# real-stanford/flingbot

Measured on AMD Instinct MI355X. Metric: sim steps/sec (64x64-particle cloth), higher is better.
Workload: dtype f32

## Files before the change

### flingbot_amd/csrc/fs_fused_grid_kernel.h

```cpp
#pragma once
#include "fs_fused_kernel.h"

#define FG_PLANE (FS_FUSED_MAX_PARTICLES * 4)
#define FG_PAD 1024
#define FG_OFF_XX FG_PAD
#define FG_OFF_X0 (FG_OFF_XX + 4 * FG_PLANE)
#define FG_OFF_CACC (FG_OFF_X0 + 3 * FG_PLANE)
#define FG_OFF_CUR (FG_OFF_CACC + FS_FUSED_CSET_CAP * 16)
#define FG_OFF_ITEMS (FG_OFF_CUR + FS_FUSED_CUR_BYTES)
#define FG_OFF_SCAN (FG_OFF_ITEMS + FS_FUSED_MAX_PARTICLES * 2)
#define FG_OFF_CSET (FG_OFF_SCAN + 64)
#define FG_OFF_CHIST (FG_OFF_CSET + FS_FUSED_CSET_CAP * 2)
#define FG_OFF_ROWL (FG_OFF_CHIST + 512)
#define FG_OFF_KZ (FG_OFF_ROWL + 1024)
#define FG_OFF_KS (FG_OFF_KZ + 1024)
#define FG_OFF_COLL (FG_OFF_KS + 1024)
#define FG_OFF_RCNT (FG_OFF_COLL + 512)
#define FG_LDS_BYTES (FG_OFF_RCNT + 512)
static_assert(FG_OFF_ROWL % 8 == 0 && (FG_OFF_KZ - FG_OFF_ROWL) % 8 == 0, "row tables are read as ds_read_b64 pairs");
static_assert((FG_OFF_COLL - FG_OFF_KS) % 256 == 0, "column tables share one address, rows as ds_read2st64_b32 offsets");
static_assert(FG_LDS_BYTES <= 160 * 1024, "grid-64 kernel: the LDS of one CU");
static_assert(FG_OFF_CACC % 16 == 0 && FG_OFF_CUR == FG_OFF_CACC + FS_FUSED_CSET_CAP * 16, "set and queue accumulators: one array");
#ifndef FG_SINGLES
#define FG_SINGLES 1
#endif
#define FG_SINGLES_LANES (FS_FUSED_THREADS - 64)
#define FG_SINGLES_ROOM ((FS_FUSED_CUR_BYTES + FS_FUSED_MAX_PARTICLES * 2) / 16)
#define FG_SINGLES_CAP (FG_SINGLES_ROOM < 2 * FG_SINGLES_LANES ? FG_SINGLES_ROOM : 2 * FG_SINGLES_LANES)
#define FG_SLOT_NONE 0xffffu
#define FG_SLOT_INLINE 0xfffeu
static_assert(FS_FUSED_CSET_CAP + FG_SINGLES_CAP <= FG_SLOT_INLINE, "slot values below the reserved ones");

#define FG_ROW(w, k) (2 * (w) + 32 * ((k) >> 1) + ((k) & 1))

template <int DZ>
__device__ __forceinline__ void fg_load_slot(unsigned a, fs_f2 &x0, fs_f2 &x1, fs_f2 &x2) {
    asm volatile("ds_read2st64_b32 %0, %1 offset0:%2 offset1:%3" : "=v"(x0) : "v"(a), "n"(DZ + 2), "n"(DZ + 3) : "memory");
    asm volatile("ds_read2st64_b32 %0, %1 offset0:%2 offset1:%3" : "=v"(x1) : "v"(a), "n"(DZ + 2 + 64), "n"(DZ + 3 + 64) : "memory");
    asm volatile("ds_read2st64_b32 %0, %1 offset0:%2 offset1:%3" : "=v"(x2) : "v"(a), "n"(DZ + 2 + 128), "n"(DZ + 3 + 128) : "memory");
}
template <int OFF>
__device__ __forceinline__ fs_f2 fg_load_rows(unsigned a) {
    static_assert(OFF >= 0 && OFF < 65536 && OFF % 8 == 0, "ds_read_b64 offset");
    fs_f2 r;
    asm volatile("ds_read_b64 %0, %1 offset:%2" : "=v"(r) : "v"(a), "n"(OFF) : "memory");
    return r;
}
template <int R0, int R1>
__device__ __forceinline__ fs_f2 fg_load_cols(unsigned a) {
    static_assert(R0 >= 0 && R0 < 256 && R1 >= 0 && R1 < 256, "ds_read2st64_b32 offsets");
    fs_f2 r;
    asm volatile("ds_read2st64_b32 %0, %1 offset0:%2 offset1:%3" : "=v"(r) : "v"(a), "n"(R0), "n"(R1) : "memory");
    return r;
}
#define FG_WAIT(N, A0, A1, A2) asm volatile("s_waitcnt lgkmcnt(" #N ")" : "+v"(A0), "+v"(A1), "+v"(A2))

#define FG_MIN_L2 1.17549435e-38f
__device__ __forceinline__ float fg_scale(float xi0, float xi1, float xi2, float xj0, float xj1, float xj2, float L, float k,
                                          float &l2) {
    const float ex = xi0 - xj0, ey = xi1 - xj1, ez = xi2 - xj2;
    l2 = fs_dot3(ex, ey, ez, ex, ey, ez);
    const float inv = __builtin_amdgcn_rsqf(l2);
    const float len = l2 * inv;
    const float C = len - L;
    return k * (C * inv);
}
__device__ __forceinline__ void fg_accum(float &d0, float &d1, float &d2, float xi0, float xi1, float xi2, float xj0, float xj1,
                                         float xj2, float sc) {
    const float ex = xi0 - xj0, ey = xi1 - xj1, ez = xi2 - xj2;
    d0 = FS_FMA(-ex, sc, d0);
    d1 = FS_FMA(-ey, sc, d1);
    d2 = FS_FMA(-ez, sc, d2);
}
__device__ __forceinline__ float fg_from_left(float v) {
    return __int_as_float(__builtin_amdgcn_update_dpp(0, __float_as_int(v), 0x138, 0xf, 0xf, true));
}
__device__ __forceinline__ float fg_from_right(float v) {
    return __int_as_float(__builtin_amdgcn_update_dpp(0, __float_as_int(v), 0x130, 0xf, 0xf, true));
}

__device__ __forceinline__ void fg_apply(const FsAcc &a, float relax, const float *rcnt, float &x0, float &x1, float &x2) {
    if (a.cnt > 0) {
        const float sc = a.cnt < 128 ? rcnt[a.cnt] : relax / (float)a.cnt;
        x0 = FS_FMA(a.d0, sc, x0); x1 = FS_FMA(a.d1, sc, x1); x2 = FS_FMA(a.d2, sc, x2);
    }
}

__global__ __launch_bounds__(FS_FUSED_THREADS) void fs_k_fused_grid64(const FsEnvDev *__restrict__ envs,
                                                                      const FsShapesDev *__restrict__ shapes, const int *ids,
                                                                      int n_steps) {
    static_assert(FS_FUSED_THREADS == 1024 && FS_FUSED_PPT == 4, "grid-64 kernel: 16 waves x 4 rows");
    extern __shared__ __attribute__((aligned(16))) char smem[];
    float *Xx = (float *)(smem + FG_OFF_XX);
    float *Xy = Xx + FS_FUSED_MAX_PARTICLES, *Xz = Xy + FS_FUSED_MAX_PARTICLES, *Xw = Xz + FS_FUSED_MAX_PARTICLES;
    float *X0x = (float *)(smem + FG_OFF_X0);
    float *X0y = X0x + FS_FUSED_MAX_PARTICLES;
    float *X0z = X0y + FS_FUSED_MAX_PARTICLES;
    unsigned short *cursor = (unsigned short *)(smem + FG_OFF_CUR);
    unsigned short *items = (unsigned short *)(smem + FG_OFF_ITEMS);
    int *wave_tot = (int *)(smem + FG_OFF_SCAN);
    float *rowL = (float *)(smem + FG_OFF_ROWL);

#ifdef FS_BLOCK_CLOCKS
    const unsigned long long tc_start = __builtin_amdgcn_s_memtime(), tr_start = __builtin_amdgcn_s_memrealtime();
#endif
#ifdef FS_TIMING
    unsigned long long ts_acc[16] = {0, 0, 0, 0, 0, 0, 0, 0, 0, 0, 0, 0, 0, 0, 0, 0};
    unsigned long long ts_last = __builtin_amdgcn_s_memtime();
#endif
    const int e = ids[blockIdx.x];
    if (e < 0) return;
    const FsEnvDev &E = envs[e];
    const FsShapesDev &sh = shapes[e];
    const FsFusedConsts c = fs_fused_consts(E, sh);
    const int n = c.n;
    const unsigned un = (unsigned)n;
    const int t = threadIdx.x, lane = t & 63, w = t >> 6;
    const int dimz = n >> 6;

    FsVec4 *const g_pos = E.pos, *const g_vel = E.vel;
    const FsVec4 *const g_rest = E.rest;
    const fs_gci g_phase = (fs_gci)E.phase;
    const fs_gi g_nlist = (fs_gi)E.nlist, g_ncount = (fs_gi)E.ncount;
    const fs_gci g_ell_j = (fs_gci)E.ell_j;
    const fs_gcf g_ell_len = (fs_gcf)E.ell_len, g_ell_k = (fs_gcf)E.ell_k;
    const fs_gcf g_L = (fs_gcf)E.g64_L;
    const int max_deg = E.max_deg;
    const fs_gcu g_near = (fs_gcu)E.restnear_w;

    int find_mode = 0;
    {
        const int ph0 = g_phase[0];
        int differs = 0;
        for (int i = t; i < n; i += FS_FUSED_THREADS) differs |= (g_phase[i] != ph0);
        if (t == 0) wave_tot[0] = 0;
        __syncthreads();
        if (differs) atomicOr(&wave_tot[0], 1);
        __syncthreads();
        const int mixed = wave_tot[0];
        __syncthreads();
        if (!mixed) {
            if (!(ph0 & FS_PHASE_SELF_COLLIDE)) find_mode = 3;
            else if (!(ph0 & FS_PHASE_SELF_COLLIDE_FILTER)) find_mode = 2;
            else if (E.restnear_ok == 2 && FS_STENCIL_FILTER) find_mode = 4;
            else if (E.restnear_ok) find_mode = 1;
        }
    }
    for (int q = t; q < FG_OFF_X0 / 4; q += FS_FUSED_THREADS) ((float *)smem)[q] = 0.0f;
    __syncthreads();
    for (int i = t; i < n; i += FS_FUSED_THREADS) {
        const FsVec4 p = fs_ld4(g_pos, i);
        Xx[i] = p.x; Xy[i] = p.y; Xz[i] = p.z; Xw[i] = p.w;
        X0x[i] = p.x; X0y[i] = p.y; X0z[i] = p.z;
    }
    if (t < 256) {
        const int r = t & 63, s = 8 + (t >> 6);
        rowL[t] = r < dimz ? g_L[(unsigned)s * un + (unsigned)(r * 64 + 2)] : 0.0f;
    }
    constexpr int XS_DX[4] = {-1, -2, +1, +2};
    constexpr int SH_DX[4] = {+1, -1, -1, +1}, SH_DZ[4] = {-1, -1, +1, +1};
    constexpr int ZS_DZ[4] = {-1, -2, +1, +2};
    float *colL = (float *)(smem + FG_OFF_COLL);
    if (t < 128) {
        const int col = t & 63, q = t >> 6;
        const int dxq = q == 0 ? -1 : -2;
        colL[t] = (unsigned)(col + dxq) < 64u ? g_L[(unsigned)q * un + (unsigned)(2 * 64 + col)] : 0.0f;
    }
    float *rcnt = (float *)(smem + FG_OFF_RCNT);
    if (t < 128) rcnt[t] = t > 0 ? c.relax / (float)t : 0.0f;
    if (t < 256) {
        const int c64 = t & 63, q = t >> 6;
        const int sdx = (q == 0 || q == 3) ? +1 : -1, sslot = q < 2 ? 2 + q : 4 + q;
        const int zdz = q < 2 ? -1 - q : q - 1;
        ((float *)(smem + FG_OFF_KS))[t] = (unsigned)(c64 + sdx) < 64u ? E.g64_kh[sslot] : 0.0f;
        ((float *)(smem + FG_OFF_KZ))[t] = (c64 < dimz && (unsigned)(c64 + zdz) < (unsigned)dimz) ? E.g64_kh[8 + q] : 0.0f;
    }
    const float kh0 = E.g64_kh[0], kh1 = E.g64_kh[1];
    unsigned nvalid = 0u;
#pragma unroll
    for (int k = 0; k < FS_FUSED_PPT; ++k) {
        const int row = FG_ROW(w, k);
        int cnt = 0;
#pragma unroll
        for (int q = 0; q < 4; ++q) {
            cnt += ((unsigned)(lane + XS_DX[q]) < 64u) ? 1 : 0;
            cnt += ((unsigned)(lane + SH_DX[q]) < 64u && (unsigned)(row + SH_DZ[q]) < (unsigned)dimz) ? 1 : 0;
            cnt += ((unsigned)(row + ZS_DZ[q]) < (unsigned)dimz) ? 1 : 0;
        }
        nvalid |= (unsigned)cnt << (8 * k);
    }
    __syncthreads();
    unsigned fastmask = 0u;
    {
        constexpr int cdx[FS_G64_SLOTS] = FS_G64_DX_LIST, cdz[FS_G64_SLOTS] = FS_G64_DZ_LIST;
#pragma unroll
        for (int k = 0; k < FS_FUSED_PPT; ++k) {
            const int row = FG_ROW(w, k), i = row * 64 + lane;
            bool differs = false;
            if (i < n) {
                const float wi = Xw[i];
                differs = !(wi > 0.0f);
#pragma unroll
                for (int q = 0; q < FS_G64_SLOTS; ++q) {
                    const bool in = (unsigned)(lane + cdx[q]) < 64u && (unsigned)(row + cdz[q]) < (unsigned)dimz;
                    if (in) differs |= Xw[i + cdz[q] * 64 + cdx[q]] != wi;
                }
            }
            if (i < n && __builtin_amdgcn_ballot_w64(differs) == 0ull) fastmask |= 1u << k;
        }
        fastmask = (unsigned)__builtin_amdgcn_readfirstlane((int)fastmask);
    }

    FS_TS(0)
#pragma unroll 1
    for (int frame = 0; frame < n_steps; ++frame) {
#pragma unroll 1
        for (int sub = 0; sub < c.substeps; ++sub) {
            for (int q = t; q < FS_FUSED_BUCKETS / 2; q += FS_FUSED_THREADS) ((unsigned *)cursor)[q] = 0u;
            FsVec4 xp[FS_FUSED_PPT];
#pragma unroll
            for (int k = 0; k < FS_FUSED_PPT; ++k) {
                const int i = t + k * FS_FUSED_THREADS;
                xp[k] = FsVec4{0.0f, 0.0f, 0.0f, 0.0f};
                if (i < n) {
                    const FsVec4 p0 = FsVec4{X0x[i], X0y[i], X0z[i], Xw[i]};
                    xp[k] = fs_fused_predict(c, p0, fs_ld4(g_vel, i));
                    fs_st4(E.x0, i, p0);
                }
            }
            __syncthreads();
            fs_fused_build_grid(c, xp, cursor, items, wave_tot, X0x, X0y, X0z);
            FS_TS(1)
            const FsFindConsts fc = {n, c.ncap, c.rad2, c.inv_rad, find_mode, E.gp_dimx, E.gp_magic};
#pragma unroll 1
            for (int qs = t; qs < n; qs += FS_FUSED_THREADS) {
                const int i = items[qs];
                const FsVec4 xi = FsVec4{X0x[qs], X0y[qs], X0z[qs], 0.0f};
                const int shape_bits = (int)(fs_shape_candidates(E.p, sh, sub, xi.x, xi.y, xi.z) << FS_SHAPE_MASK_SHIFT);
                if (find_mode == 4) {
                    FsNearWords none;
#pragma unroll
                    for (int q = 0; q < 8; ++q) none.w[q] = 0xffffffffu;
                    g_ncount[i] = fs_fused_find_neighbors<true>(fc, i, xi, (fs_lcus)cursor, (fs_lcus)items, g_phase, g_rest, g_nlist,
                                                                none, (fs_lus)(smem + FG_OFF_XX) + t, (fs_lcf)X0x) | shape_bits;
                    continue;
                }
                FsNearWords near;
#pragma unroll
                for (int q = 0; q < 8; ++q) near.w[q] = find_mode == 1 ? g_near[(unsigned)q * un + (unsigned)i] : 0xffffffffu;
                g_ncount[i] = (find_mode == 3 ? 0
                                              : fs_fused_find_neighbors<false>(fc, i, xi, (fs_lcus)cursor, (fs_lcus)items, g_phase,
                                                                               g_rest, g_nlist, near,
                                                                               (fs_lus)(smem + FG_OFF_XX) + t, (fs_lcf)X0x)) |
                              shape_bits;
            }
            FS_TS(2)
            __syncthreads();
            FS_TS(3)
#pragma unroll
            for (int k = 0; k < FS_FUSED_PPT; ++k) {
                const int i = t + k * FS_FUSED_THREADS;
                if (i < n) {
                    Xx[i] = xp[k].x; Xy[i] = xp[k].y; Xz[i] = xp[k].z; Xw[i] = xp[k].w;
                    const FsVec4 p0 = fs_ld4(E.x0, i);
                    X0x[i] = p0.x; X0y[i] = p0.y; X0z[i] = p0.z;
                } else {
                    Xx[i] = 0.0f; Xy[i] = 0.0f; Xz[i] = 0.0f; Xw[i] = 0.0f;
                }
            }

            unsigned short *cset = (unsigned short *)(smem + FG_OFF_CSET);
            FsVec4 *cacc = (FsVec4 *)(smem + FG_OFF_CACC);
            int *chist = (int *)(smem + FG_OFF_CHIST);
            if (t < 128) chist[t] = 0;
            int *nsingles = (int *)(smem + FG_OFF_SCAN);
            if (t == 0) *nsingles = 0;
            __syncthreads();
            int ccls[FS_FUSED_PPT];
#pragma unroll
            for (int k = 0; k < FS_FUSED_PPT; ++k) {
                const int i = FG_ROW(w, k) * 64 + lane;
                int cc = 0;
                if (i < n && Xw[i] > 0.0f) cc = g_ncount[i] & FS_NCOUNT_MASK;
                ccls[k] = cc > 96 ? 96 : cc;
                if (ccls[k] > 0) atomicAdd(&chist[ccls[k]], 1);
            }
            __syncthreads();
            fs_fused_count_offsets(chist, t);
            __syncthreads();
            FsVec4 *squeue = cacc + FS_FUSED_CSET_CAP;
            unsigned long long slotpack = ~0ull;
#pragma unroll
            for (int k = 0; k < FS_FUSED_PPT; ++k) {
                if (ccls[k] > 0) {
                    const int i = FG_ROW(w, k) * 64 + lane;
                    unsigned slot = FG_SLOT_INLINE;
                    const int pos = atomicAdd(&chist[ccls[k]], 1);
                    if (pos < FS_FUSED_CSET_CAP) {
                        cset[pos] = (unsigned short)i;
                        slot = (unsigned)pos;
                    }
#if FG_SINGLES
                    else if (ccls[k] <= 16) {
                        const int sp = atomicAdd(nsingles, 1);
                        if (sp < FG_SINGLES_CAP) {
                            slot = (unsigned)(FS_FUSED_CSET_CAP + sp);
                            squeue[sp].w = __int_as_float(i | (g_nlist[i] << 12) | ((ccls[k] - 1) << 28));
                        }
                    }
#endif
                    slotpack = (slotpack & ~(0xffffull << (16 * k))) | ((unsigned long long)slot << (16 * k));
                }
            }
            __syncthreads();
            const int csize = chist[0] < FS_FUSED_CSET_CAP ? chist[0] : FS_FUSED_CSET_CAP;
            const int n_singles = *nsingles < FG_SINGLES_CAP ? *nsingles : FG_SINGLES_CAP;
            const int i2 = t < csize ? (int)cset[t] : -1;
            int cnt2 = 0, cj2[FS_FUSED_PREFETCH_CAND];
#pragma unroll
            for (int q = 0; q < FS_FUSED_PREFETCH_CAND; ++q) cj2[q] = 0;
            if (i2 >= 0) {
                cnt2 = g_ncount[i2] & FS_NCOUNT_MASK;
#pragma unroll
                for (int q = 0; q < FS_FUSED_PREFETCH_CAND; ++q) cj2[q] = g_nlist[(unsigned)q * un + (unsigned)i2];
            }
            static_assert(FG_SINGLES_CAP <= 2 * FG_SINGLES_LANES, "two queue entries per lane");
            unsigned qw0 = 0u, qw1 = 0u;
#if FG_SINGLES
            if (t >= 64 && t - 64 < n_singles) qw0 = (unsigned)__float_as_int(squeue[t - 64].w);
            if (t >= 64 && t - 64 + FG_SINGLES_LANES < n_singles) qw1 = (unsigned)__float_as_int(squeue[t - 64 + FG_SINGLES_LANES].w);
            __syncthreads();
#endif

            FS_TS(4)
#pragma unroll 1
            for (int it = 0; it < c.iters; ++it) {
                unsigned cpack = 0u;
                float rx[FS_FUSED_PPT], ry[FS_FUSED_PPT], rz[FS_FUSED_PPT];
#pragma unroll
                for (int q = 0; q < FS_FUSED_PPT; ++q) { rx[q] = 0.0f; ry[q] = 0.0f; rz[q] = 0.0f; }
#ifdef FG_UNROLL_PAIRS
#pragma unroll
#else
#pragma unroll 1
#endif
                for (int pr = 0; pr < 2; ++pr) {
                    const int rowP = FG_ROW(w, 2 * pr);
                    const int iP_raw = rowP * 64 + lane, iQ_raw = iP_raw + 64;
                    const bool haveP = rowP < dimz, haveQ = rowP + 1 < dimz;
                    const int iP = haveP ? iP_raw : 0, iQ = haveQ ? iQ_raw : 0;
                    const bool fast = haveQ && ((fastmask >> (2 * pr)) & 3u) == 3u;
                    const fs_f2 xi0 = fs_f2{Xx[iP], Xx[iQ]}, xi1 = fs_f2{Xy[iP], Xy[iQ]}, xi2 = fs_f2{Xz[iP], Xz[iQ]};
                    const fs_f2 wi = fs_f2{Xw[iP], Xw[iQ]};
                    FsAcc aP, aQ;
                    bool exact = !fast;
                    if (fast) {
                        unsigned aLane = (unsigned)(lane * 4);
                        asm volatile("" : "+v"(aLane));
                        const unsigned am2 = (unsigned)(FG_OFF_XX + ((rowP - 2) * 64 - 2) * 4) + aLane;
                        const unsigned am1 = am2 + 4u, a00 = am2 + 8u, ap1 = am2 + 12u, ap2 = am2 + 16u;
                        constexpr int SH_SLOT[4] = {2, 3, 6, 7};
                        float sLP[2], sLQ[4];
#pragma unroll
                        for (int q = 0; q < 2; ++q) sLP[q] = g_L[(unsigned)SH_SLOT[q] * un + (unsigned)iP];
#pragma unroll
                        for (int q = 0; q < 4; ++q) sLQ[q] = g_L[(unsigned)SH_SLOT[q] * un + (unsigned)iQ];
                        const unsigned aRow = (unsigned)(FG_OFF_ROWL + rowP * 4), aCol = (unsigned)FG_OFF_KS + aLane;
                        constexpr int CL_ROW = (FG_OFF_COLL - FG_OFF_KS) / 256;
                        fs_f2 cL = fg_load_cols<CL_ROW, CL_ROW + 1>(aCol);
                        const unsigned aKP = rowP >= 1 ? aCol : aLane;
                        const unsigned aKQ = rowP + 2 < dimz ? aCol : aLane;
                        fs_f2 kP23 = fg_load_cols<0, 1>(aKP);
                        fs_f2 kQ23 = fg_load_cols<0, 1>(aCol);
#define FG_KX(q) ((unsigned)(lane + XS_DX[q]) < 64u ? (q == 0 ? kh0 : kh1) : 0.0f)
                        float dP0 = 0.0f, dP1 = 0.0f, dP2 = 0.0f, dQ0 = 0.0f, dQ1 = 0.0f, dQ2 = 0.0f, mP = 1.0f, mQ = 1.0f;
                        fs_f2 u0, u1, u2, v0, v1, v2;
                        float l2a, l2b, l2c, l2d;
                        fg_load_slot<0>(am1, u0, u1, u2);
                        fg_load_slot<0>(am2, v0, v1, v2);
                        asm volatile("s_waitcnt lgkmcnt(3)"
                                     : "+v"(cL), "+v"(kP23), "+v"(kQ23), "+v"(u0), "+v"(u1), "+v"(u2));
                        const float scP0 = fg_scale(xi0.x, xi1.x, xi2.x, u0.x, u1.x, u2.x, cL.x, FG_KX(0), l2a);
                        const float scQ0 = fg_scale(xi0.y, xi1.y, xi2.y, u0.y, u1.y, u2.y, cL.x, FG_KX(0), l2b);
                        fg_accum(dP0, dP1, dP2, xi0.x, xi1.x, xi2.x, u0.x, u1.x, u2.x, scP0);
                        fg_accum(dQ0, dQ1, dQ2, xi0.y, xi1.y, xi2.y, u0.y, u1.y, u2.y, scQ0);
                        __builtin_amdgcn_sched_barrier(0);
                        fg_load_slot<-1>(ap1, u0, u1, u2);
                        FG_WAIT(3, v0, v1, v2);
                        const float scP1 = fg_scale(xi0.x, xi1.x, xi2.x, v0.x, v1.x, v2.x, cL.y, FG_KX(1), l2c);
                        const float scQ1 = fg_scale(xi0.y, xi1.y, xi2.y, v0.y, v1.y, v2.y, cL.y, FG_KX(1), l2d);
                        fg_accum(dP0, dP1, dP2, xi0.x, xi1.x, xi2.x, v0.x, v1.x, v2.x, scP1);
                        fg_accum(dQ0, dQ1, dQ2, xi0.y, xi1.y, xi2.y, v0.y, v1.y, v2.y, scQ1);
                        mP = fminf(fminf(mP, l2a), l2c);
                        mQ = fminf(fminf(mQ, l2b), l2d);
                        __builtin_amdgcn_sched_barrier(0);
                        fg_load_slot<-1>(am1, v0, v1, v2);
                        FG_WAIT(3, u0, u1, u2);
                        const float scQ2 = fg_scale(xi0.y, xi1.y, xi2.y, u0.y, u1.y, u2.y, sLQ[0], kQ23.x, l2b);
                        {
                            const float sc = fg_scale(xi0.x, xi1.x, xi2.x, u0.x, u1.x, u2.x, sLP[0], kP23.x, l2a);
                            fg_accum(dP0, dP1, dP2, xi0.x, xi1.x, xi2.x, u0.x, u1.x, u2.x, sc);
                        }
                        fg_accum(dQ0, dQ1, dQ2, xi0.y, xi1.y, xi2.y, u0.y, u1.y, u2.y, scQ2);
                        __builtin_amdgcn_sched_barrier(0);
                        fg_load_slot<0>(ap1, u0, u1, u2);
                        FG_WAIT(3, v0, v1, v2);
                        const float scQ3 = fg_scale(xi0.y, xi1.y, xi2.y, v0.y, v1.y, v2.y, sLQ[1], kQ23.y, l2d);
                        {
                            const float sc = fg_scale(xi0.x, xi1.x, xi2.x, v0.x, v1.x, v2.x, sLP[1], kP23.y, l2c);
                            fg_accum(dP0, dP1, dP2, xi0.x, xi1.x, xi2.x, v0.x, v1.x, v2.x, sc);
                        }
                        fg_accum(dQ0, dQ1, dQ2, xi0.y, xi1.y, xi2.y, v0.y, v1.y, v2.y, scQ3);
                        mP = fminf(fminf(mP, l2a), l2c);
                        mQ = fminf(fminf(mQ, l2b), l2d);
                        __builtin_amdgcn_sched_barrier(0);
                        fg_load_slot<0>(ap2, v0, v1, v2);
                        FG_WAIT(3, u0, u1, u2);
                        fg_accum(dP0, dP1, dP2, xi0.x, xi1.x, xi2.x, u0.x, u1.x, u2.x, fg_from_right(scP0));
                        fg_accum(dQ0, dQ1, dQ2, xi0.y, xi1.y, xi2.y, u0.y, u1.y, u2.y, fg_from_right(scQ0));
                        __builtin_amdgcn_sched_barrier(0);
                        fs_f2 kQ67 = fg_load_cols<2, 3>(aKQ);
                        fg_load_slot<+1>(am1, u0, u1, u2);
                        FG_WAIT(3, v0, v1, v2);
                        fg_accum(dP0, dP1, dP2, xi0.x, xi1.x, xi2.x, v0.x, v1.x, v2.x, fg_from_right(fg_from_right(scP1)));
                        fg_accum(dQ0, dQ1, dQ2, xi0.y, xi1.y, xi2.y, v0.y, v1.y, v2.y, fg_from_right(fg_from_right(scQ1)));
                        __builtin_amdgcn_sched_barrier(0);
                        fg_load_slot<+1>(ap1, v0, v1, v2);
                        asm volatile("s_waitcnt lgkmcnt(3)" : "+v"(kQ67), "+v"(u0), "+v"(u1), "+v"(u2));
                        fg_accum(dP0, dP1, dP2, xi0.x, xi1.x, xi2.x, u0.x, u1.x, u2.x, fg_from_left(scQ2));
                        {
                            const float sc = fg_scale(xi0.y, xi1.y, xi2.y, u0.y, u1.y, u2.y, sLQ[2], kQ67.x, l2a);
                            fg_accum(dQ0, dQ1, dQ2, xi0.y, xi1.y, xi2.y, u0.y, u1.y, u2.y, sc);
                        }
                        __builtin_amdgcn_sched_barrier(0);
                        constexpr int KZ = FG_OFF_KZ - FG_OFF_ROWL;
                        fs_f2 zL[4], zK[4];
                        zL[0] = fg_load_rows<0>(aRow); zK[0] = fg_load_rows<KZ>(aRow);
                        zL[1] = fg_load_rows<256>(aRow); zK[1] = fg_load_rows<KZ + 256>(aRow);
                        fg_load_slot<-1>(a00, u0, u1, u2);
                        asm volatile("s_waitcnt lgkmcnt(3)"
                                     : "+v"(zL[0]), "+v"(zK[0]), "+v"(zL[1]), "+v"(zK[1]), "+v"(v0), "+v"(v1), "+v"(v2));
                        fg_accum(dP0, dP1, dP2, xi0.x, xi1.x, xi2.x, v0.x, v1.x, v2.x, fg_from_right(scQ3));
                        {
                            const float sc = fg_scale(xi0.y, xi1.y, xi2.y, v0.y, v1.y, v2.y, sLQ[3], kQ67.y, l2b);
                            fg_accum(dQ0, dQ1, dQ2, xi0.y, xi1.y, xi2.y, v0.y, v1.y, v2.y, sc);
                        }
                        mQ = fminf(fminf(mQ, l2a), l2b);
                        __builtin_amdgcn_sched_barrier(0);
                        fg_load_slot<-2>(a00, v0, v1, v2);
                        FG_WAIT(3, u0, u1, u2);
                        const float scQ8 = fg_scale(xi0.y, xi1.y, xi2.y, u0.y, u1.y, u2.y, zL[0].y, zK[0].y, l2b);
                        {
                            const float sc = fg_scale(xi0.x, xi1.x, xi2.x, u0.x, u1.x, u2.x, zL[0].x, zK[0].x, l2a);
                            fg_accum(dP0, dP1, dP2, xi0.x, xi1.x, xi2.x, u0.x, u1.x, u2.x, sc);
                        }
                        fg_accum(dQ0, dQ1, dQ2, xi0.y, xi1.y, xi2.y, u0.y, u1.y, u2.y, scQ8);
                        __builtin_amdgcn_sched_barrier(0);
                        zL[2] = fg_load_rows<512>(aRow); zK[2] = fg_load_rows<KZ + 512>(aRow);
                        zL[3] = fg_load_rows<768>(aRow); zK[3] = fg_load_rows<KZ + 768>(aRow);
                        fg_load_slot<+1>(a00, u0, u1, u2);
                        asm volatile("s_waitcnt lgkmcnt(3)"
                                     : "+v"(zL[2]), "+v"(zK[2]), "+v"(zL[3]), "+v"(zK[3]), "+v"(v0), "+v"(v1), "+v"(v2));
                        {
                            const float sc = fg_scale(xi0.x, xi1.x, xi2.x, v0.x, v1.x, v2.x, zL[1].x, zK[1].x, l2c);
                            const float sd = fg_scale(xi0.y, xi1.y, xi2.y, v0.y, v1.y, v2.y, zL[1].y, zK[1].y, l2d);
                            fg_accum(dP0, dP1, dP2, xi0.x, xi1.x, xi2.x, v0.x, v1.x, v2.x, sc);
                            fg_accum(dQ0, dQ1, dQ2, xi0.y, xi1.y, xi2.y, v0.y, v1.y, v2.y, sd);
                        }
                        mP = fminf(fminf(mP, l2a), l2c);
                        mQ = fminf(fminf(mQ, l2b), l2d);
                        __builtin_amdgcn_sched_barrier(0);
                        fg_load_slot<+2>(a00, v0, v1, v2);
                        FG_WAIT(3, u0, u1, u2);
                        fg_accum(dP0, dP1, dP2, xi0.x, xi1.x, xi2.x, u0.x, u1.x, u2.x, scQ8);
                        {
                            const float sd = fg_scale(xi0.y, xi1.y, xi2.y, u0.y, u1.y, u2.y, zL[2].y, zK[2].y, l2c);
                            fg_accum(dQ0, dQ1, dQ2, xi0.y, xi1.y, xi2.y, u0.y, u1.y, u2.y, sd);
                        }
                        __builtin_amdgcn_sched_barrier(0);
                        FG_WAIT(0, v0, v1, v2);
                        {
                            const float sc = fg_scale(xi0.x, xi1.x, xi2.x, v0.x, v1.x, v2.x, zL[3].x, zK[3].x, l2a);
                            const float sd = fg_scale(xi0.y, xi1.y, xi2.y, v0.y, v1.y, v2.y, zL[3].y, zK[3].y, l2b);
                            fg_accum(dP0, dP1, dP2, xi0.x, xi1.x, xi2.x, v0.x, v1.x, v2.x, sc);
                            fg_accum(dQ0, dQ1, dQ2, xi0.y, xi1.y, xi2.y, v0.y, v1.y, v2.y, sd);
                        }
                        mP = fminf(mP, l2a);
                        mQ = fminf(fminf(mQ, l2c), l2b);
                        __builtin_amdgcn_sched_barrier(0);
#undef FG_KX
                        exact = __builtin_amdgcn_ballot_w64(mP < FG_MIN_L2 || mQ < FG_MIN_L2) != 0ull;
                        aP = FsAcc{dP0, dP1, dP2, (int)((nvalid >> (16 * pr)) & 0xffu)};
                        aQ = FsAcc{dQ0, dQ1, dQ2, (int)((nvalid >> (16 * pr + 8)) & 0xffu)};
                    }
                    if (exact) {
                        aP = FsAcc{0.0f, 0.0f, 0.0f, 0};
                        aQ = FsAcc{0.0f, 0.0f, 0.0f, 0};
                        if (haveP && wi.x > 0.0f)
                            for (int s = 0; s < max_deg; ++s) {
                                const int j = g_ell_j[(unsigned)s * un + (unsigned)iP];
                                if (j < 0) break;
                                fs_spring(aP, xi0.x, xi1.x, xi2.x, wi.x, FsVec4{Xx[j], Xy[j], Xz[j], Xw[j]},
                                          g_ell_len[(unsigned)s * un + (unsigned)iP], g_ell_k[(unsigned)s * un + (unsigned)iP]);
                            }
                        if (haveQ && wi.y > 0.0f)
                            for (int s = 0; s < max_deg; ++s) {
                                const int j = g_ell_j[(unsigned)s * un + (unsigned)iQ];
                                if (j < 0) break;
                                fs_spring(aQ, xi0.y, xi1.y, xi2.y, wi.y, FsVec4{Xx[j], Xy[j], Xz[j], Xw[j]},
                                          g_ell_len[(unsigned)s * un + (unsigned)iQ], g_ell_k[(unsigned)s * un + (unsigned)iQ]);
                            }
                    }
                    FS_TS(5)
#pragma unroll
                    for (int h = 0; h < 2; ++h) {
                        const int i = h == 0 ? iP : iQ;
                        FsAcc a = h == 0 ? aP : aQ;
                        const unsigned myslot = (unsigned)(slotpack >> (16 * (2 * pr + h))) & 0xffffu;
                        if (myslot < FG_SLOT_INLINE) {
                            cacc[myslot] = FsVec4{a.d0, a.d1, a.d2, __int_as_float(a.cnt)};
                        } else if (myslot == FG_SLOT_INLINE) {
                            const float xi0s = h == 0 ? xi0.x : xi0.y, xi1s = h == 0 ? xi1.x : xi1.y, xi2s = h == 0 ? xi2.x : xi2.y;
                            const float wis = h == 0 ? wi.x : wi.y;
                            const float ri0 = xi0s - X0x[i], ri1 = xi1s - X0y[i], ri2 = xi2s - X0z[i];
                            const int cnt = g_ncount[i] & FS_NCOUNT_MASK;
#pragma unroll 1
                            for (int sq = 0; sq < cnt; ++sq) {
                                const int j = g_nlist[(unsigned)sq * un + (unsigned)i];
                                const FsVec4 xj = FsVec4{Xx[j], Xy[j], Xz[j], Xw[j]};
                                fs_particle_contact(a, xi0s, xi1s, xi2s, wis, ri0, ri1, ri2, xj, xj.x - X0x[j], xj.y - X0y[j],
                                                    xj.z - X0z[j], c.restd, c.restd2, c.mu_p);
                            }
                        }
#pragma unroll
                        for (int q = FS_FUSED_PPT - 1; q > 0; --q) { rx[q] = rx[q - 1]; ry[q] = ry[q - 1]; rz[q] = rz[q - 1]; }
                        rx[0] = a.d0; ry[0] = a.d1; rz[0] = a.d2;
                        cpack = (cpack << 8) | (unsigned)a.cnt;
                    }
                    FS_TS(6)
                }
                __syncthreads();
                FS_TS(7)
                unsigned smk[FS_FUSED_PPT];
#pragma unroll
                for (int k = 0; k < FS_FUSED_PPT; ++k) {
                    const int i = FG_ROW(w, k) * 64 + lane;
                    unsigned ic = i < n ? (unsigned)i : 0u;
                    asm volatile("" : "+v"(ic));
                    smk[k] = (unsigned)g_ncount[ic] >> FS_SHAPE_MASK_SHIFT;
                }
                if (i2 >= 0) {
                    const float xi0 = Xx[i2], xi1 = Xy[i2], xi2 = Xz[i2], wi = Xw[i2];
                    const FsVec4 pa = cacc[t];
                    FsAcc a = {pa.x, pa.y, pa.z, __float_as_int(pa.w)};
                    const float ri0 = xi0 - X0x[i2], ri1 = xi1 - X0y[i2], ri2 = xi2 - X0z[i2];
                    int cjt[FS_FUSED_PREFETCH_CAND];
#pragma unroll
                    for (int q = 0; q < FS_FUSED_PREFETCH_CAND; ++q) cjt[q] = cj2[q];
                    for (int s0 = 0; s0 < cnt2; s0 += FS_FUSED_PREFETCH_CAND) {
                        int cn[FS_FUSED_PREFETCH_CAND];
#pragma unroll
                        for (int q = 0; q < FS_FUSED_PREFETCH_CAND; ++q) {
                            const int sn = s0 + FS_FUSED_PREFETCH_CAND + q;
                            cn[q] = sn < cnt2 ? g_nlist[(unsigned)sn * un + (unsigned)i2] : 0;
                        }
#pragma unroll 1
                        for (int q = 0; q < FS_FUSED_PREFETCH_CAND && s0 + q < cnt2; ++q) {
                            const int j = cjt[0];
#pragma unroll
                            for (int r = 0; r + 1 < FS_FUSED_PREFETCH_CAND; ++r) cjt[r] = cjt[r + 1];
                            const FsVec4 xj = FsVec4{Xx[j], Xy[j], Xz[j], Xw[j]};
                            fs_particle_contact(a, xi0, xi1, xi2, wi, ri0, ri1, ri2, xj, xj.x - X0x[j], xj.y - X0y[j],
                                                xj.z - X0z[j], c.restd, c.restd2, c.mu_p);
                        }
#pragma unroll
                        for (int q = 0; q < FS_FUSED_PREFETCH_CAND; ++q) cjt[q] = cn[q];
                    }
                    cacc[t] = FsVec4{a.d0, a.d1, a.d2, __int_as_float(a.cnt)};
                }
#if FG_SINGLES
#pragma unroll 1
                for (int r = 0, q = t - 64; q >= 0 && q < n_singles; ++r, q += FG_SINGLES_LANES) {
                    const unsigned word = r == 0 ? qw0 : qw1;
                    const int i = (int)(word & 0xfffu), more = (int)(word >> 28);
                    int j = (int)((word >> 12) & 0xfffu);
                    int jn = more > 0 ? g_nlist[un + (unsigned)i] : 0;
                    const FsVec4 pa = squeue[q];
                    FsAcc a = {pa.x, pa.y, pa.z, __float_as_int(pa.w)};
                    const float xi0 = Xx[i], xi1 = Xy[i], xi2 = Xz[i], wi = Xw[i];
                    const float ri0 = xi0 - X0x[i], ri1 = xi1 - X0y[i], ri2 = xi2 - X0z[i];
#pragma unroll 1
                    for (int sq = 0; sq <= more; ++sq) {
                        const FsVec4 xj = FsVec4{Xx[j], Xy[j], Xz[j], Xw[j]};
                        fs_particle_contact(a, xi0, xi1, xi2, wi, ri0, ri1, ri2, xj, xj.x - X0x[j], xj.y - X0y[j], xj.z - X0z[j], c.restd,
                                            c.restd2, c.mu_p);
                        j = jn;
                        if (sq + 2 <= more) jn = g_nlist[(unsigned)(sq + 2) * un + (unsigned)i];
                    }
                    squeue[q] = FsVec4{a.d0, a.d1, a.d2, __int_as_float(a.cnt)};
                }
#endif
                FS_TS(8)
                __syncthreads();
                FS_TS(9)
#pragma unroll 1
                for (int k = 0; k < FS_FUSED_PPT; ++k) {
                    const int i = FG_ROW(w, k) * 64 + lane;
                    const unsigned myslot = (unsigned)(slotpack >> (16 * k)) & 0xffffu;
                    FsAcc a = {rx[FS_FUSED_PPT - 1], ry[FS_FUSED_PPT - 1], rz[FS_FUSED_PPT - 1], (int)(cpack >> 8 * (FS_FUSED_PPT - 1))};
                    const unsigned smask = smk[0];
#pragma unroll
                    for (int q = FS_FUSED_PPT - 1; q > 0; --q) { rx[q] = rx[q - 1]; ry[q] = ry[q - 1]; rz[q] = rz[q - 1]; }
#pragma unroll
                    for (int q = 0; q + 1 < FS_FUSED_PPT; ++q) smk[q] = smk[q + 1];
                    cpack <<= 8;
                    if (i < n) {
                        const float wi = Xw[i];
                        if (wi > 0.0f) {
                            if (myslot < FG_SLOT_INLINE) {
                                const FsVec4 pa = cacc[myslot];
                                a = FsAcc{pa.x, pa.y, pa.z, __float_as_int(pa.w)};
                            }
                            float xi0 = Xx[i], xi1 = Xy[i], xi2 = Xz[i];
                            const float ri0 = xi0 - X0x[i], ri1 = xi1 - X0y[i], ri2 = xi2 - X0z[i];
                            fs_fused_shape_contacts(a, c, E.p, sh, sub, smask, xi0, xi1, xi2, ri0, ri1, ri2);
                            fg_apply(a, c.relax, rcnt, xi0, xi1, xi2);
                            Xx[i] = xi0; Xy[i] = xi1; Xz[i] = xi2;
                        }
                    }
                }
                __syncthreads();
                FS_TS(10)
            }
            for (int i = t; i < n; i += FS_FUSED_THREADS) {
                const FsVec4 xf = FsVec4{Xx[i], Xy[i], Xz[i], Xw[i]};
                FsVec4 p0 = FsVec4{X0x[i], X0y[i], X0z[i], xf.w};
                FsVec4 v = fs_ld4(g_vel, i);
                fs_fused_finalize(c, p0, v, xf);
                fs_st4(g_vel, i, v);
                X0x[i] = p0.x; X0y[i] = p0.y; X0z[i] = p0.z;
            }
        }
    }
    for (int i = t; i < n; i += FS_FUSED_THREADS) fs_st4(g_pos, i, FsVec4{X0x[i], X0y[i], X0z[i], Xw[i]});
#ifdef FS_BLOCK_CLOCKS
    if (t == 0) {
        const unsigned long long tc_total = __builtin_amdgcn_s_memtime() - tc_start, tr_end = __builtin_amdgcn_s_memrealtime();
        const fs_gi out = g_nlist + 95u * un;
        out[0] = (int)(unsigned)tc_total; out[1] = (int)(unsigned)(tc_total >> 32);
        out[2] = (int)(unsigned)tr_start; out[3] = (int)(unsigned)tr_end;
    }
#endif
#ifdef FS_TIMING
    FS_TS(11)
    if (blockIdx.x == 0 && (t & 63) == 0)
        printf("TS wave %2d: init %llu grid %llu find %llu findwait %llu cset %llu springs %llu park %llu bar1 %llu contact %llu bar2 %llu finish+bar3 %llu final %llu\n",
               t >> 6, ts_acc[0], ts_acc[1], ts_acc[2], ts_acc[3], ts_acc[4], ts_acc[5], ts_acc[6], ts_acc[7], ts_acc[8], ts_acc[9], ts_acc[10],
               ts_acc[11]);
#endif
}
```

Measured before the change: 131,300.

## Process particle pairs in contact/apply loop and split slot packing into 32-bit words

```diff
diff --git a/flingbot_amd/csrc/fs_fused_grid_kernel.h b/flingbot_amd/csrc/fs_fused_grid_kernel.h
--- a/flingbot_amd/csrc/fs_fused_grid_kernel.h
+++ b/flingbot_amd/csrc/fs_fused_grid_kernel.h
@@ -289,7 +289,7 @@
             fs_fused_count_offsets(chist, t);
             __syncthreads();
             FsVec4 *squeue = cacc + FS_FUSED_CSET_CAP;
-            unsigned long long slotpack = ~0ull;
+            unsigned slotw[2] = {~0u, ~0u};
 #pragma unroll
             for (int k = 0; k < FS_FUSED_PPT; ++k) {
                 if (ccls[k] > 0) {
@@ -309,7 +309,7 @@
                         }
                     }
 #endif
-                    slotpack = (slotpack & ~(0xffffull << (16 * k))) | ((unsigned long long)slot << (16 * k));
+                    slotw[k >> 1] = (slotw[k >> 1] & ~(0xffffu << (16 * (k & 1)))) | (slot << (16 * (k & 1)));
                 }
             }
             __syncthreads();
@@ -336,9 +336,9 @@
 #pragma unroll 1
             for (int it = 0; it < c.iters; ++it) {
                 unsigned cpack = 0u;
-                float rx[FS_FUSED_PPT], ry[FS_FUSED_PPT], rz[FS_FUSED_PPT];
-#pragma unroll
-                for (int q = 0; q < FS_FUSED_PPT; ++q) { rx[q] = 0.0f; ry[q] = 0.0f; rz[q] = 0.0f; }
+                float rold[2][3], rnew[2][3];
+#pragma unroll
+                for (int q = 0; q < 6; ++q) { rold[q / 3][q % 3] = 0.0f; rnew[q / 3][q % 3] = 0.0f; }
 #ifdef FG_UNROLL_PAIRS
 #pragma unroll
 #else
@@ -512,11 +512,12 @@
                             }
                     }
                     FS_TS(5)
+                    const unsigned slw = pr == 0 ? slotw[0] : slotw[1];
 #pragma unroll
                     for (int h = 0; h < 2; ++h) {
                         const int i = h == 0 ? iP : iQ;
-                        FsAcc a = h == 0 ? aP : aQ;
-                        const unsigned myslot = (unsigned)(slotpack >> (16 * (2 * pr + h))) & 0xffffu;
+                        FsAcc &a = h == 0 ? aP : aQ;
+                        const unsigned myslot = h == 0 ? (slw & 0xffffu) : (slw >> 16);
                         if (myslot < FG_SLOT_INLINE) {
                             cacc[myslot] = FsVec4{a.d0, a.d1, a.d2, __int_as_float(a.cnt)};
                         } else if (myslot == FG_SLOT_INLINE) {
@@ -532,11 +533,12 @@
                                                     xj.z - X0z[j], c.restd, c.restd2, c.mu_p);
                             }
                         }
-#pragma unroll
-                        for (int q = FS_FUSED_PPT - 1; q > 0; --q) { rx[q] = rx[q - 1]; ry[q] = ry[q - 1]; rz[q] = rz[q - 1]; }
-                        rx[0] = a.d0; ry[0] = a.d1; rz[0] = a.d2;
-                        cpack = (cpack << 8) | (unsigned)a.cnt;
-                    }
+                    }
+#pragma unroll
+                    for (int q = 0; q < 3; ++q) { rold[0][q] = rnew[0][q]; rold[1][q] = rnew[1][q]; }
+                    rnew[0][0] = aP.d0; rnew[0][1] = aP.d1; rnew[0][2] = aP.d2;
+                    rnew[1][0] = aQ.d0; rnew[1][1] = aQ.d1; rnew[1][2] = aQ.d2;
+                    cpack = (cpack << 16) | ((unsigned)aP.cnt << 8) | (unsigned)aQ.cnt;
                     FS_TS(6)
                 }
                 __syncthreads();
@@ -604,30 +606,65 @@
                 __syncthreads();
                 FS_TS(9)
 #pragma unroll 1
-                for (int k = 0; k < FS_FUSED_PPT; ++k) {
-                    const int i = FG_ROW(w, k) * 64 + lane;
-                    const unsigned myslot = (unsigned)(slotpack >> (16 * k)) & 0xffffu;
-                    FsAcc a = {rx[FS_FUSED_PPT - 1], ry[FS_FUSED_PPT - 1], rz[FS_FUSED_PPT - 1], (int)(cpack >> 8 * (FS_FUSED_PPT - 1))};
-                    const unsigned smask = smk[0];
-#pragma unroll
-                    for (int q = FS_FUSED_PPT - 1; q > 0; --q) { rx[q] = rx[q - 1]; ry[q] = ry[q - 1]; rz[q] = rz[q - 1]; }
-#pragma unroll
-                    for (int q = 0; q + 1 < FS_FUSED_PPT; ++q) smk[q] = smk[q + 1];
-                    cpack <<= 8;
-                    if (i < n) {
-                        const float wi = Xw[i];
-                        if (wi > 0.0f) {
-                            if (myslot < FG_SLOT_INLINE) {
-                                const FsVec4 pa = cacc[myslot];
-                                a = FsAcc{pa.x, pa.y, pa.z, __float_as_int(pa.w)};
-                            }
-                            float xi0 = Xx[i], xi1 = Xy[i], xi2 = Xz[i];
-                            const float ri0 = xi0 - X0x[i], ri1 = xi1 - X0y[i], ri2 = xi2 - X0z[i];
-                            fs_fused_shape_contacts(a, c, E.p, sh, sub, smask, xi0, xi1, xi2, ri0, ri1, ri2);
-                            fg_apply(a, c.relax, rcnt, xi0, xi1, xi2);
-                            Xx[i] = xi0; Xy[i] = xi1; Xz[i] = xi2;
-                        }
-                    }
+                for (int pr = 0; pr < 2; ++pr) {
+                    const int iP = FG_ROW(w, 2 * pr) * 64 + lane;
+                    const unsigned slw = pr == 0 ? slotw[0] : slotw[1];
+                    FsAcc a[2];
+                    unsigned sm[2];
+                    bool act[2];
+                    float x0[2], x1[2], x2[2], r0[2], r1[2], r2[2];
+                    int n_planes = c.n_planes, n_shapes = c.n_shapes;
+                    asm volatile("" : "+s"(n_planes), "+s"(n_shapes));
+#pragma unroll
+                    for (int h = 0; h < 2; ++h) {
+                        const int i = iP + 64 * h;
+                        const unsigned myslot = h == 0 ? (slw & 0xffffu) : (slw >> 16);
+                        act[h] = (i < n) & (Xw[i] > 0.0f);
+                        a[h] = FsAcc{rold[h][0], rold[h][1], rold[h][2], (int)(h == 0 ? cpack >> 24 : (cpack >> 16) & 0xffu)};
+                        if (act[h] && myslot < FG_SLOT_INLINE) {
+                            const FsVec4 pa = cacc[myslot];
+                            a[h] = FsAcc{pa.x, pa.y, pa.z, __float_as_int(pa.w)};
+                        }
+                        sm[h] = act[h] ? (pr == 0 ? smk[h] : smk[2 + h]) : 0u;
+                        x0[h] = Xx[i]; x1[h] = Xy[i]; x2[h] = Xz[i];
+                        r0[h] = x0[h] - X0x[i]; r1[h] = x1[h] - X0y[i]; r2[h] = x2[h] - X0z[i];
+                    }
+#pragma unroll
+                    for (int q = 0; q < 3; ++q) { rold[0][q] = rnew[0][q]; rold[1][q] = rnew[1][q]; }
+                    cpack <<= 16;
+#pragma unroll
+                    for (int h = 0; h < 2; ++h) {
+                        int q = 0;
+                        if (n_planes == 1) {
+                            if (sm[h] & 1u)
+                                fs_plane_contact(a[h], x0[h], x1[h], x2[h], r0[h], r1[h], r2[h], c.pl0, c.pl1, c.pl2, c.pl3, c.cd, c.mu_s,
+                                                 c.mu_k);
+                            q = 1;
+                        }
+                        for (; q < n_planes; ++q)
+                            if ((sm[h] >> q) & 1u)
+                                fs_plane_contact(a[h], x0[h], x1[h], x2[h], r0[h], r1[h], r2[h], E.p.planes[q][0], E.p.planes[q][1],
+                                                 E.p.planes[q][2], E.p.planes[q][3], c.cd, c.mu_s, c.mu_k);
+                    }
+                    if (n_shapes != 0 && __builtin_amdgcn_ballot_w64(((sm[0] | sm[1]) >> FS_SHAPE_SPHERE_BIT) != 0u) != 0ull) {
+                        const float S = (float)c.substeps;
+#pragma unroll
+                        for (int h = 0; h < 2; ++h)
+                            for (int q = 0; q < n_shapes; ++q)
+                                if ((sm[h] >> (FS_SHAPE_SPHERE_BIT + q)) & 1u) {
+                                    float c0, c1, c2, s0, s1, s2;
+                                    fs_shape_sweep(sh, q, sub, S, c0, c1, c2, s0, s1, s2);
+                                    fs_sphere_contact(a[h], x0[h], x1[h], x2[h], r0[h], r1[h], r2[h], c0, c1, c2, sh.pos[q].w, s0, s1, s2,
+                                                      c.cd, c.mu_s, c.mu_k);
+                                }
+                    }
+#pragma unroll
+                    for (int h = 0; h < 2; ++h)
+                        if (act[h]) {
+                            const int i = iP + 64 * h;
+                            fg_apply(a[h], c.relax, rcnt, x0[h], x1[h], x2[h]);
+                            Xx[i] = x0[h]; Xy[i] = x1[h]; Xz[i] = x2[h];
+                        }
                 }
                 __syncthreads();
                 FS_TS(10)
```

Result: faster. 135,200, median of 6 (+2.9%).
